# shichaoy/cube_slam

Hardware: AMD Instinct MI355X
Metric: frames/sec front-end (ORB extract + LSD+LBD lines + cuboid: Canny+DT+sweep+score+select) @640x480 (higher is better)
Workload: dtype f64

## Files before the change

cube_slam_amd/csrc/cuboid.hip:

```cpp
#include "common.h"

#include <algorithm>
#include <array>
#include <climits>
#include <cmath>
#include <vector>

namespace {

constexpr int ROLL_CAP = 8;
constexpr int RP_CAP = ROLL_CAP * ROLL_CAP;
constexpr int SWEEP_HB = 1024;
constexpr int NMS_TW = 64, NMS_TH = 16;
constexpr int DT_INIT = INT_MAX >> 2;
constexpr int DT_HV = 62587;
constexpr int DT_DIAG = 89738;
constexpr size_t DT_SERIAL_ROW_BYTES = 2 * 4 * sizeof(int);
constexpr double PI = 3.14159265358979323846;
constexpr int SC_LDS_BYTES = 160 * 1024;
constexpr int SC_LUT_N = 1024;
constexpr int SC_CTRL_BYTES = 64;
constexpr int SC_MAP_OFF = SC_CTRL_BYTES + 2048;
constexpr int SC_MAP_ENTRIES = (SC_LDS_BYTES - SC_MAP_OFF) / 2;
constexpr float SC_ESC_D = 244.0f;
// ... 737 lines not shown
                if (!BWD) tmp[((long)i * C + k) * 64 + lane] = t;
                else lbuf[(rows_done & 1) * WC + jcol[k]] = (float)t * scale;
            }
            if (BWD) { flush_store(); rows_done++; }
        }
    }
    if (BWD && rows_done > 0) {
        const float *lb = lbuf + ((rows_done - 1) & 1) * WC;
#pragma unroll
        for (int q = 0; q < C; q++) ob[q] = lb[q * 64 + lane];
        oi = 0;
        flush_store();
    }
}
template <int C>
__global__ void __launch_bounds__(256) cuboid_dt_wave(const Unit *units, int n_units, const uint8_t *emap, int *tmp_arena, const long *tmp_off, float *dist) {
    const int u = blockIdx.x * 4 + (threadIdx.x >> 6);
    if (u >= n_units) return;
    const Unit &U = units[u];
    int *tmp = tmp_arena + tmp_off[u];
    __shared__ float s_line[4][2 * 64 * C];
    dt_wave_pass<C, false>(U, emap + U.pix_off, tmp, nullptr, nullptr);
    __builtin_amdgcn_fence(__ATOMIC_SEQ_CST, "workgroup");
    dt_wave_pass<C, true>(U, nullptr, tmp, dist + U.pix_off, s_line[threadIdx.x >> 6]);
}

struct VPEntry { double vp[6]; double ang[6]; };

__global__ void __launch_bounds__(256) cuboid_vp(const Unit *units, const UnitDyn *ud, const FrameDyn *fd, const CamRP *cam, const double *yaw,
                                                 Opts o, const double *mangle, const double *mmid, VPEntry *vpt) {
    const Unit &U = units[blockIdx.y];
    const FrameDyn &D = fd[U.frame];
    const int n_rp = D.n_roll * D.n_pitch;
    const int e = blockIdx.x * 256 + threadIdx.x;
    if (e >= n_rp * D.n_yaw) return;
    const int rp = e / D.n_yaw, yi = e % D.n_yaw;
    const CamRP &C = cam[(long)U.frame * RP_CAP + rp];
    const double y = yaw[(long)U.frame * o.yaw_cap + yi];
    const double cy = cos(y), sy = sin(y);
    VPEntry E;
    {
        const double d[3][3] = {{cy, sy, 0}, {-sy, cy, 0}, {0, 0, 1}};
        for (int k = 0; k < 3; k++) {
            double r[3];
            for (int i = 0; i < 3; i++) {
                double s = C.KinvR[i * 3 + 0] * d[k][0];
                s = s + C.KinvR[i * 3 + 1] * d[k][1];
                s = s + C.KinvR[i * 3 + 2] * d[k][2];
                r[i] = s;
// ... 863 lines not shown
                U.roi_w = U.roi_r - U.roi_x; U.roi_h = U.roi_b - U.roi_y;
                if (U.roi_w <= 0 || U.roi_h <= 0 || U.roi_x + U.roi_w > width || U.roi_y + U.roi_h > height) { ctx->err = "box ROI outside the image"; return CS_ERR_BAD_ARG; }
                U.pix_off = P.pix_total; P.pix_total += ((long)U.roi_w * U.roi_h + 63) / 64 * 64;
                U.hyp_cap = rp_cap * o.yaw_cap * U.n_tops * 2;
                U.hyp_off = P.hyp_total; P.hyp_total += ((long)U.hyp_cap + 63) / 64 * 64;
                U.vp_off = (int)P.vp_total; P.vp_total += (long)rp_cap * o.yaw_cap;
                U.line_off = (int)P.line_rows; P.line_rows += std::min(fi[f].n_lines, CS_MAX_ROI_LINES);
                U.nms_off = P.n_nms; P.n_nms += ((U.roi_w + NMS_TW - 1) / NMS_TW) * ((U.roi_h + NMS_TH - 1) / NMS_TH);
                U.cc_off = P.n_cc; P.n_cc += (int)(((long)U.roi_w * U.roi_h + 4095) / 4096);
                U.hb_off = P.n_hb; P.n_hb += (U.hyp_cap + SWEEP_HB - 1) / SWEEP_HB;
                P.max_roi_w = std::max(P.max_roi_w, U.roi_w);
                P.max_cc_blocks = std::max(P.max_cc_blocks, (int)(((long)U.roi_w * U.roi_h + 4095) / 4096));
                P.units.push_back(U);
            }
        }
    P.max_vp_blocks = (rp_cap * o.yaw_cap + 255) / 256;
    P.n_units = (int)P.units.size();
    if (P.vp_total > INT_MAX || P.line_rows > INT_MAX) return CS_ERR_CAPACITY;
    return CS_OK;
}
static void plan_derived(Plan &P, int score_G) {
    const size_t n = P.units.size();
    P.wgmap.resize((size_t)P.n_nms + P.n_cc + P.n_hb);
    for (size_t u = 0; u < n; u++) {
        const Unit &U = P.units[u];
        const int e_nms = u + 1 < n ? P.units[u + 1].nms_off : P.n_nms, e_cc = u + 1 < n ? P.units[u + 1].cc_off : P.n_cc, e_hb = u + 1 < n ? P.units[u + 1].hb_off : P.n_hb;
        for (int k = U.nms_off; k < e_nms; k++) P.wgmap[(size_t)k] = (int)u;
        for (int k = U.cc_off; k < e_cc; k++) P.wgmap[(size_t)P.n_nms + k] = (int)u;
        for (int k = U.hb_off; k < e_hb; k++) P.wgmap[(size_t)P.n_nms + P.n_cc + k] = (int)u;
    }
    static const int CS_[] = {4, 5, 6, 8, 10, 12, 16, 20};
// ... 290 lines not shown
    for (const FrameInfo &fi_ : b->fi) ul_cap = std::max(ul_cap, std::min(fi_.n_lines, CS_MAX_ROI_LINES));
    const bool fork = !ctx->timing;
    hipStream_t side = ctx->stream;
    SideBranch branch{ctx};
    if (fork) {
        CS_HIP(ctx, ctx->aux_get(&side));
        if (!b->ev_fork) CS_HIP(ctx, hipEventCreateWithFlags(&b->ev_fork, hipEventDisableTiming));
        if (!b->ev_join) CS_HIP(ctx, hipEventCreateWithFlags(&b->ev_join, hipEventDisableTiming));
        CS_HIP(ctx, hipEventRecord(b->ev_fork, ctx->stream));
        branch.side = side;
        CS_HIP(ctx, hipStreamWaitEvent(side, b->ev_fork, 0));
    }
    CS_LAUNCH_ON(ctx, side, "cuboid_frame_prep", cuboid_frame_prep, dim3(b->n_frames), dim3(64), 0, b->d_fi, b->d_fd, b->d_cam, b->d_yaw, b->cal, b->o, b->d_lines_in, b->d_lines_al);
    CS_LAUNCH_ON(ctx, side, "cuboid_unit_lines", cuboid_unit_lines, dim3(U), dim3(64), sizeof(double) * 5 * (size_t)ul_cap, b->d_units, b->d_ud, b->d_fi, b->d_lines_al, b->d_mlines,
                 b->d_mangle, b->d_mmid, b->d_status, ul_cap);
    CS_LAUNCH_ON(ctx, side, "cuboid_vp", cuboid_vp, dim3(b->max_vp_blocks, U), dim3(256), 0, b->d_units, b->d_ud, b->d_fd, b->d_cam, b->d_yaw, b->o, b->d_mangle, b->d_mmid, b->d_vp);
    CS_HIP(ctx, hipGetLastError());
    if (fork) { CS_HIP(ctx, hipEventRecord(b->ev_join, side)); branch.joined = b->ev_join; }
    CS_HIP(ctx, hipMemsetAsync(b->d_emap, 0, (size_t)b->pix_total, ctx->stream));
    CS_LAUNCH(ctx, "cuboid_canny_nms", cuboid_canny_nms, dim3(b->n_nms), dim3(256), 0, b->d_units, b->d_wgmap, b->d_gray, b->W, b->H, b->d_emap,
              b->d_lab, b->o.canny_low, b->o.canny_high);
    CS_LAUNCH(ctx, "cuboid_canny_cc_local", cuboid_canny_cc_local, dim3(b->n_cc), dim3(256), 0, b->d_units, b->d_wgmap + b->n_nms, b->d_emap, b->d_lab);
    if (b->max_cc_blocks > 1)
        CS_LAUNCH(ctx, "cuboid_canny_cc_border", cuboid_canny_cc_border, dim3(U, 4), dim3(256), 0, b->d_units, b->d_emap, b->d_lab);
    CS_LAUNCH(ctx, "cuboid_canny_cc", cuboid_canny_cc, dim3(b->n_cc), dim3(256), 0, b->d_units, b->d_wgmap + b->n_nms, b->d_emap, b->d_lab);
    if (b->dt_C) {
        const dim3 g((U + 3) / 4), t(256);
        switch (b->dt_C) {
#define DTW_(c) case c: CS_LAUNCH(ctx, "cuboid_dt", cuboid_dt_wave<c>, g, t, 0, b->d_units, U, b->d_emap, b->d_dttmp, b->d_dttmp_off, b->d_dist); break;
            DTW_(4) DTW_(5) DTW_(6) DTW_(8) DTW_(10) DTW_(12) DTW_(16) DTW_(20)
#undef DTW_
        }
    } else if (b->max_roi_w <= 1024) {
        CS_LAUNCH(ctx, "cuboid_dt", cuboid_dt_block, dim3(U), dim3(64 * ((b->max_roi_w + 63) / 64)), 0, b->d_units, b->d_emap, b->d_dist);
    } else {
        const int wbuf = b->max_roi_w + 2;
        CS_LAUNCH(ctx, "cuboid_dt", cuboid_dt, dim3((U + 3) / 4), dim3(256), (size_t)wbuf * DT_SERIAL_ROW_BYTES, b->d_units, U, b->d_emap, b->d_dist, wbuf);
    }
    CS_HIP(ctx, branch.join());
    CS_HIP(ctx, hipMemsetAsync(b->d_vcount, 0, sizeof(int) * 2 * (size_t)U, ctx->stream));
    CS_LAUNCH(ctx, "cuboid_sweep_filter", cuboid_sweep_filter, dim3(b->n_hb), dim3(256), 0, b->d_units, b->d_wgmap + b->n_nms + b->n_cc, b->d_fd, b->o, b->d_vp,
              b->d_flag, b->d_vcount, b->d_vlist);
// ... 202 lines not shown
```

cube_slam_amd/csrc/lsd.hip:

```cpp
#include "common.h"
#include "glibc_sincosf.h"
#include "lsd_regions.h"

#include <cfloat>
#include <chrono>
#include <cmath>
#include <mutex>
#include <omp.h>
#include <vector>

namespace {
constexpr double NOTDEF = -1024.0, PI_ = 3.1415926535897932384626433832795, DEG_TO_RADS = PI_ / 180;
constexpr float NOTDEF_DEG = -1024.0f;
constexpr int KH = 3;

__host__ __device__ inline float fast_atan2f_(float y, float x) {
    const float p1 = 0.9997878412794807f * (float)(180 / PI_), p3 = -0.3258083974640975f * (float)(180 / PI_), p5 = 0.1555786518463281f * (float)(180 / PI_),
                p7 = -0.04432655554792128f * (float)(180 / PI_);
    float ax = fabsf(x), ay = fabsf(y), a, c, c2;
    if (ax >= ay) { c = ay / (ax + (float)DBL_EPSILON); c2 = c * c; a = (((p7 * c2 + p5) * c2 + p3) * c2 + p1) * c; }
    else { c = ax / (ay + (float)DBL_EPSILON); c2 = c * c; a = 90.f - (((p7 * c2 + p5) * c2 + p3) * c2 + p1) * c; }
    if (x < 0) a = 180.f - a;
    if (y < 0) a = 360.f - a;
    return a;
// ... 94 lines not shown
        }
    };
#pragma unroll
    for (int u = 0; u < AHEAD; u++) fetch(u, ca[u], cc[u]);
    for (int k0 = 0; k0 < total; k0 += G) {
#pragma unroll
        for (int u = 0; u < G; u++)
            if (k0 + u < total) { fetch(k0 + u + AHEAD, ca[(u + AHEAD) % G], cc[(u + AHEAD) % G]); row(k0 + u, u, ca[u], cc[u]); }
    }
    if (dy_last == h - 1 && y0 + LSD_ROWS >= h) {
        if (mine) { const long o = (frame_px + h - 1) * w + dx; modgrad[o] = 0; angles[o] = NOTDEF_DEG; }
        if (lane == 0) seg_cnt[(frame_px + h - 1) * seg_stride + strip] = 0;
    }
}
static_assert(EMIT_STRIPS == 4, "lsd_scan_blocks reads a segment's strip counts as one int4");
__global__ void __launch_bounds__(1024) lsd_scan_blocks(const int4 *in, int n, int *out, int *block_tot) {
    __shared__ int ws[16];
    const int i = blockIdx.x * 1024 + threadIdx.x, lane = threadIdx.x & 63, wave = threadIdx.x >> 6;
    int v = 0;
    if (i < n) { const int4 q = in[i]; v = q.x + q.y + q.z + q.w; }
    const int sc = wave_incl_scan(v, lane);
    if (lane == 63) ws[wave] = sc;
    __syncthreads();
    int base = 0;
    for (int k = 0; k < wave; k++) base += ws[k];
    if (i < n) out[i] = base + sc - v;
    if (threadIdx.x == 1023) block_tot[blockIdx.x] = base + sc;
}
__global__ void __launch_bounds__(1024) lsd_scan_add(int *out, int n, const int *block_tot) {
    __shared__ int ws[16];
    int part = 0;
    for (int k = threadIdx.x; k < (int)blockIdx.x; k += 1024) part += block_tot[k];
    for (int d = 32; d > 0; d >>= 1) part += __shfl_xor(part, d);
    if ((threadIdx.x & 63) == 0) ws[threadIdx.x >> 6] = part;
    __syncthreads();
    int base = 0;
    for (int k = 0; k < 16; k++) base += ws[k];
    const int i = blockIdx.x * 1024 + threadIdx.x;
    if (i < n) out[i] += base;
    if (blockIdx.x == gridDim.x - 1 && threadIdx.x == 0) out[n] = base + block_tot[blockIdx.x];
}
template <bool PIX> __global__ void __launch_bounds__(EMIT_COLS) lsd_emit(const double *modgrad, const float *angles, int w, int h, const int *seg_base, int *c_addr, float *c_deg, float2 *c_cs, double *c_mod, float *fre ) {
    constexpr int NW = EMIT_COLS / 64, LW = EMIT_COLS + 2;
    __shared__ float s_ang[(EMIT_ROWS + 2) * LW];
    __shared__ int s_list[EMIT_ROWS * EMIT_COLS], s_need[PIX ? EMIT_ROWS * EMIT_COLS : 1];
    __shared__ int wc[EMIT_ROWS][NW], s_base[EMIT_ROWS], n_need;
    const int tid = threadIdx.x, x0 = blockIdx.x * EMIT_COLS, y0 = blockIdx.y * EMIT_ROWS;
    const long frame_row = (long)blockIdx.z * h;
    for (int i = tid; i < (EMIT_ROWS + 2) * LW; i += EMIT_COLS) {
        const int yy = y0 - 1 + i / LW, xx = x0 - 1 + i % LW;
        s_ang[i] = xx >= 0 && xx < w && yy >= 0 && yy < h ? angles[(frame_row + yy) * w + xx] : NOTDEF_DEG;
    }
    if (tid < EMIT_ROWS && y0 + tid < h) s_base[tid] = seg_base[(frame_row + y0 + tid) * gridDim.x + blockIdx.x];
    if (tid == 0) n_need = 0;
// ... 424 lines not shown
}

static int lsd_run(cs_ctx *ctx, cs_lsd *l, int with_lbd) {
    if (!ctx || !l || l->n_frames < 1) return CS_ERR_BAD_ARG;
    CS_HIP(ctx, hipSetDevice(ctx->device));
    const int W = l->W, H = l->H, w = l->w, h = l->h, F = l->n_frames;
    l->have_desc = false;
    const char *mode = getenv("CUBESLAM_LSD_REGIONS");
    if (!mode || !*mode) mode = l->region_stage == CS_LSD_REGIONS_HOST ? "host" : l->region_stage == CS_LSD_REGIONS_WAVE_PER_FRAME ? "seq" : l->region_stage == CS_LSD_REGIONS_BACKLOG ? "wlk" : (F >= 512 ? "seq" : "host");
    const int grp_p = strcmp(mode, "wlk") == 0 ? 65 : 0;
    const bool device_mode = strcmp(mode, "seq") == 0 || grp_p;
    l->scaled_kept = !device_mode;
    const int nbx = l->nbx, nsx = l->nsx, n_seg = F * h * nbx;
    CS_LAUNCH(ctx, "lsd_gradient", lsd_maps, dim3(nsx * ((h + LSD_ROWS - 1) / LSD_ROWS), 1, F), dim3(64), 0, l->d_gray, W, H, w, h, l->gk, (MapTabs{l->d_xofs, l->d_yofs, l->d_ax, l->d_ay}), l->threshold,
              l->d_mod, l->d_ang, l->d_seg_cnt, nbx * EMIT_STRIPS, device_mode ? (double *)nullptr : l->d_scaled);
    const int nblk = (n_seg + 1023) / 1024;
    CS_LAUNCH(ctx, "lsd_scan", lsd_scan_blocks, dim3(nblk), dim3(1024), 0, reinterpret_cast<const int4 *>(l->d_seg_cnt), n_seg, l->d_seg_base, l->d_blk_tot);
    CS_LAUNCH(ctx, "lsd_scan", lsd_scan_add, dim3(nblk), dim3(1024), 0, l->d_seg_base, n_seg, l->d_blk_tot);
    l->frame_base.assign((size_t)F + 1, 0);
    CS_HIP(ctx, hipMemcpy2DAsync(l->frame_base.data(), sizeof(int), l->d_seg_base, sizeof(int) * (size_t)h * nbx, sizeof(int), (size_t)F + 1, hipMemcpyDeviceToHost, ctx->stream));
    CS_HIP(ctx, hipStreamSynchronize(ctx->stream));
    const size_t total = (size_t)l->frame_base[F];
    int r;
    if (total > l->ccap) {
        void *old[] = {l->d_caddr, l->d_cdeg, l->d_ccs, l->d_cmod};
        for (void *q : old) cs_dfree(ctx, q);
        l->d_caddr = nullptr; l->d_cdeg = nullptr; l->d_ccs = nullptr; l->d_cmod = nullptr; l->ccap = 0;
        const size_t cap = total + total / 16 + 4096;
        r = cs_dalloc(ctx, &l->d_caddr, cap); if (r) return r;
        r = cs_dalloc(ctx, &l->d_cdeg, cap); if (r) return r;
        r = cs_dalloc(ctx, &l->d_ccs, cap); if (r) return r;
        l->ccap = cap;
    }
// ... 160 lines not shown
    std::vector<float> ax((size_t)l->w * 2), ay((size_t)l->h * 2);
    auto fl = [](double v) { int i = (int)v; return i - (i > v); };
    for (int dx = 0; dx < l->w; dx++) { float fx = (float)((dx + 0.5) * sx - 0.5); int s = fl(fx); fx -= s; if (s < 0) { fx = 0; s = 0; } if (s >= width - 1) { fx = 0; s = width - 1; } xofs[dx] = s; ax[dx * 2] = 1.f - fx; ax[dx * 2 + 1] = fx; }
    for (int dy = 0; dy < l->h; dy++) { float fy = (float)((dy + 0.5) * sx - 0.5); int s = fl(fy); fy -= s; if (s < 0) { fy = 0; s = 0; } if (s >= height - 1) { fy = 0; s = height - 1; } yofs[dy] = s; ay[dy * 2] = 1.f - fy; ay[dy * 2 + 1] = fy; }
    const size_t N = (size_t)width * height * max_frames, n = (size_t)l->w * l->h * max_frames;
#define A_(call) do { int r__ = (call); if (r__ != CS_OK) { cs_lsd_destroy(ctx, l); return r__; } } while (0)
    l->pix_bytes = (n * 4 + 64 + 255) / 256 * 256;
    A_(cs_dalloc(ctx, &l->d_gray, N)); A_(cs_dalloc(ctx, &l->d_tmp, N + n)); l->d_scaled = l->d_tmp + N;
    A_(cs_dalloc(ctx, &l->d_mod, n)); A_(cs_dalloc(ctx, &l->d_ang, n));
    A_(cs_dalloc(ctx, &l->d_xofs, xofs.size())); A_(cs_dalloc(ctx, &l->d_yofs, yofs.size())); A_(cs_dalloc(ctx, &l->d_ax, ax.size())); A_(cs_dalloc(ctx, &l->d_ay, ay.size()));
    l->nsx = (l->w + LSD_COLS - 1) / LSD_COLS; l->nbx = (l->nsx + EMIT_STRIPS - 1) / EMIT_STRIPS;
    for (int d0 = 0; d0 < l->w; d0 += LSD_COLS)
        if (std::min(xofs[std::min(d0 + LSD_COLS, l->w - 1)] + 1, width - 1) - xofs[d0] >= LSD_SPAN) { cs_lsd_destroy(ctx, l); return CS_ERR_BAD_ARG; }
    const size_t n_seg = (size_t)max_frames * l->h * l->nbx;
    A_(cs_dalloc(ctx, &l->d_seg_cnt, n_seg * EMIT_STRIPS)); A_(cs_dalloc(ctx, &l->d_seg_base, n_seg + 1));
    A_(cs_dalloc(ctx, &l->d_blk_tot, (n_seg + 1023) / 1024 + 1));
    { hipError_t e = hipMemsetAsync(l->d_seg_cnt, 0, n_seg * EMIT_STRIPS * sizeof(int), ctx->stream); if (e != hipSuccess) { cs_lsd_destroy(ctx, l); return CS_ERR_HIP; } }
    A_(cs_h2d(ctx, l->d_xofs, xofs.data(), xofs.size())); A_(cs_h2d(ctx, l->d_yofs, yofs.data(), yofs.size()));
    A_(cs_h2d(ctx, l->d_ax, ax.data(), ax.size())); A_(cs_h2d(ctx, l->d_ay, ay.data(), ay.size()));
#undef A_
    { hipError_t e = hipStreamSynchronize(ctx->stream); if (e != hipSuccess) { cs_lsd_destroy(ctx, l); return CS_ERR_HIP; } }
    *out = l;
    return CS_OK;
}

int cs_lsd_detect(cs_ctx *ctx, cs_lsd *l, const uint8_t *gray, int n_frames, int stride, cs_keyline *out, int cap, int *counts) {
    if (!out || !counts || cap < 1) return CS_ERR_BAD_ARG;
    int r = lsd_upload(ctx, l, gray, n_frames, stride); if (r) return r;
    r = lsd_run(ctx, l, 0); if (r) return r;
    int status = CS_OK;
    for (int f = 0; f < n_frames; f++) {
// ... 128 lines not shown
```

cube_slam_amd/csrc/lsd_regions.hip:

```cpp
#include "common.h"

#include <cfloat>
#include <climits>
#include <cmath>
#include <vector>

#include "lsd_regions.h"
#include "lsd_rg_seq.h"
#include "lsd_rg_wlk.h"

namespace {
constexpr int PAD_PX = 272, PAD_LIST = 272, PAD_RECT = 34;
constexpr double PI_ = rg::PI_, LOG_EPS = 0.0, LSD_SCALE = 0.8;
struct AngMap { int w, h; const float *deg; };

__device__ __forceinline__ double rg_log_gamma_windschitl(double x) { return 0.918938533204673 + (x - 0.5) * log(x) - x + 0.5 * x * log(x * sinh(1 / x) + 1 / (810.0 * pow(x, 6.0))); }
__device__ double rg_log_gamma(double x) {
    if (x > 15.0) return rg_log_gamma_windschitl(x);
    const double q[7] = {75122.6331530, 80916.6278952, 36308.2951477, 8687.24529705, 1168.92649479, 83.8676043424, 2.50662827511};
    double a = (x + 0.5) * log(x + 5.5) - (x + 5.5), b = 0;
    for (int n = 0; n < 7; ++n) { a -= log(x + double(n)); b += q[n] * pow(x, double(n)); }
    return a + log(b);
}
#ifndef RG_IMPROVE_WAVES
#ifndef RG_IMPROVE_WAVES
#define RG_IMPROVE_WAVES 3
#endif
#endif
constexpr int LG_N = 32768;
__global__ void __launch_bounds__(256) lsd_rg_lgamma_table(double *t) { const int i = blockIdx.x * 256 + threadIdx.x; if (i < LG_N) t[i] = i > 0 ? rg_log_gamma(double(i)) : 0.0; }
__device__ __forceinline__ double rg_lgam_int(int x, const double *lgt) { return x < LG_N ? lgt[x] : rg_log_gamma_windschitl(double(x)); }
__device__ double rg_nfa(int n, int k, double p, double LOG_NT, const double *lgt) {
    if (n == 0 || k == 0) return -LOG_NT;
    if (n == k) return -LOG_NT - double(n) * log10(p);
    const double p_term = p / (1 - p);
    const double log1term = (double(n) + 1) - rg_lgam_int(k + 1, lgt) - rg_lgam_int(n - k + 1, lgt) + double(k) * log(p) + double(n - k) * log(1.0 - p);
    double term = exp(log1term);
    const double RELATIVE_ERROR_FACTOR = 100.0;
    auto double_equal = [&](double a, double b) { if (a == b) return true; double abs_diff = fabs(a - b), aa = fabs(a), bb = fabs(b); double abs_max = aa > bb ? aa : bb; if (abs_max < DBL_MIN) abs_max = DBL_MIN; return (abs_diff / abs_max) <= (RELATIVE_ERROR_FACTOR * DBL_EPSILON); };
    if (double_equal(term, 0)) { if (k > n * p) return -log1term / 2.30258509299404568402 - LOG_NT; else return -LOG_NT; }
    double bin_tail = term;
    const double tolerance = 0.1;
    for (int i = k + 1; i <= n; ++i) {
        const double bin_term = double(n - i + 1) / double(i), mult_term = bin_term * p_term;
        term *= mult_term;
        bin_tail += term;
        if (bin_term < 1) {
// ... 239 lines not shown
        return;
    }
    for (;;) {
        int t = 0;
        if (lane == 0) t = rgw::lds_add(&mail.head, 1);
        t = __builtin_amdgcn_readfirstlane(t);
        bool quit = false;
        while (__builtin_amdgcn_readfirstlane(rgw::lds_ld(&mail.ring_tick[t % NS])) != t + 1) {
            if (__builtin_amdgcn_readfirstlane(rgw::lds_ld(&mail.walkers_done)) == WK && __builtin_amdgcn_readfirstlane(rgw::lds_ld(&mail.tail)) <= t) { quit = true; break; }
            __builtin_amdgcn_s_sleep(4);
        }
        if (quit) break;
        rgw::serve_ticket<rgs::Wave, NS>(B, mail, t);
    }
}
__global__ void __launch_bounds__(1024) lsd_rg_cand_scan(const int *cand_cnt, int F, int *cand_base) {
    __shared__ int part[1024];
    const int t = threadIdx.x, per = (F + 1023) / 1024;
    int sum = 0;
    for (int k = 0; k < per; k++) { const int f = t * per + k; if (f < F) sum += cand_cnt[f]; }
    part[t] = sum;
    __syncthreads();
    for (int d = 1; d < 1024; d <<= 1) { const int v = t >= d ? part[t - d] : 0; __syncthreads(); part[t] += v; __syncthreads(); }
    int run = part[t] - sum;
    for (int k = 0; k < per; k++) { const int f = t * per + k; if (f < F) { cand_base[f] = run; run += cand_cnt[f]; } }
    if (t == 1023) cand_base[F] = part[1023];
}
constexpr uint8_t HAS_DEFERRED = 2;
template <class E, bool REDO> __device__ __forceinline__ void lsd_rg_improve_body(const SeqParams &P, const int *cand_base, int n_cand, const E &nfa, float4 *line, uint8_t *has, unsigned long long *counters) {
    const int base = (blockIdx.x * 4 + (threadIdx.x >> 6)) * 8, lane = threadIdx.x & 63, grp = lane >> 3, sub = lane & 7;
    if (base >= n_cand) return;
    const int mine = base + grp;
    bool on = mine < n_cand;
    if (REDO) {
        on = on && has[mine] == HAS_DEFERRED;
        if (!__any(on)) return;
    }
    auto frame_of = [&](int wv) { int lo = 0, hi = P.F; while (hi - lo > 1) { const int mid = (lo + hi) >> 1; if (cand_base[mid] <= wv) lo = mid; else hi = mid; } return lo; };
    auto load_rect = [&](int wv, int f, rg::Rect &rec) {
        const double *o = P.rect + (size_t)f * P.rect_stride + (size_t)(wv - cand_base[f]) * 12;
        rec.x1 = o[0]; rec.y1 = o[1]; rec.x2 = o[2]; rec.y2 = o[3]; rec.width = o[4]; rec.x = o[5]; rec.y = o[6]; rec.theta = o[7]; rec.dx = o[8]; rec.dy = o[9]; rec.prec = o[10]; rec.p = o[11];
    };
    auto emit = [&](int wv, rg::Rect rec, double log_nfa) {
        const bool ok = log_nfa > LOG_EPS;
        if (ok) {
            rec.x1 += 0.5; rec.y1 += 0.5; rec.x2 += 0.5; rec.y2 += 0.5;
            rec.x1 /= LSD_SCALE; rec.y1 /= LSD_SCALE; rec.x2 /= LSD_SCALE; rec.y2 /= LSD_SCALE;
            line[wv] = make_float4(float(rec.x1), float(rec.y1), float(rec.x2), float(rec.y2));
        }
        has[wv] = ok ? 1 : 0;
    };
    const int f1 = frame_of(on ? mine : n_cand - 1);
// ... 4 lines not shown
    {
        RectSpan S; S.set(r1, P.h);
        const float *deg = P.ang + (size_t)f1 * P.w * P.h;
        int tot = 0, alg[1] = {0};
        if (on)
            for (int y = S.y_first + sub; y <= S.y_hi; y += 8) {
                int lx, rx;
                if (!S.row(y, P.w, lx, rx)) continue;
                tot += rx - lx + 1;
                rg_row_count<1>(deg + (size_t)y * P.w, lx, rx, 0, 1, r1.theta, &r1.prec, alg);
            }
        for (int off = 1; off < 8; off <<= 1) { tot += __shfl_xor(tot, off); alg[0] += __shfl_xor(alg[0], off); }
        log1 = nfa(tot, alg[0], r1.p, miss1);
    }
    if (on && sub == 0) { if (miss1) has[mine] = HAS_DEFERRED; else if (log1 > LOG_EPS) emit(mine, r1, log1); }
    int n_deferred = __popcll(__ballot(on && sub == 0 && miss1));
    unsigned long long todo = __ballot(on && sub == 0 && !miss1 && !(log1 > LOG_EPS));
    while (todo) {
        const int l = __ffsll((long long)todo) - 1;
        todo &= todo - 1;
        const int wv = base + (l >> 3), f = __shfl(f1, l);
        const double first = __shfl(log1, l);
        rg::Rect rec;
        load_rect(wv, f, rec);
        const AngMap Fr = {P.w, P.h, P.ang + (size_t)f * P.w * P.h};
        bool missed = false;
        const double log_nfa = rg_rect_improve(Fr, rec, nfa, lane, first, missed);
        if (missed) { n_deferred++; if (lane == 0) has[wv] = HAS_DEFERRED; }
        else if (lane == 0) emit(wv, rec, log_nfa);
    }
    if (!REDO && lane == 0) atomicAdd(counters, (unsigned long long)(min(8, n_cand - base) - n_deferred) | (unsigned long long)n_deferred << 32);
}
__global__ void __launch_bounds__(256) __attribute__((amdgpu_waves_per_eu(4, 4))) lsd_rg_improve(SeqParams P, const int *cand_base, int n_cand, const double *nfa_table, int nfa_nmax, float4 *line, uint8_t *has, unsigned long long *counters) {
    lsd_rg_improve_body<NfaTable, false>(P, cand_base, n_cand, NfaTable{nfa_table, nfa_nmax}, line, has, counters);
}
__global__ void __launch_bounds__(256) __attribute__((amdgpu_waves_per_eu(RG_IMPROVE_WAVES, RG_IMPROVE_WAVES))) lsd_rg_improve_deferred(SeqParams P, const int *cand_base, int n_cand, const double *lgt, float4 *line, uint8_t *has) {
    lsd_rg_improve_body<NfaDirect, true>(P, cand_base, n_cand, NfaDirect{rg_log_nt(P.w, P.h), lgt}, line, has, nullptr);
}
__global__ void __launch_bounds__(256) lsd_rg_nfa_probe(const int *t, int m, const double *nfa_table, int nfa_nmax, int w, int h, const double *lgt, double *out) {
    const int i = blockIdx.x * 256 + threadIdx.x;
    if (i >= m) return;
    const int n = t[3 * i], k = t[3 * i + 1], j = t[3 * i + 2];
    const double p = ldexp(1.0, -(3 + j));
    bool miss = false;
    const double v = NfaTable{nfa_table, nfa_nmax}(n, k, p, miss);
    out[2 * i] = miss ? __longlong_as_double(0x7ff8000000000000LL) : v;
    out[2 * i + 1] = rg_nfa(n, k, p, rg_log_nt(w, h), lgt);
}
}

struct LsdSeq {
    int F = 0, w = 0, h = 0; int cand_cap = 0; size_t cap_lines = 0;
    float *d_pix = nullptr; bool pix_borrowed = false;
    rgl::Ent *d_elist = nullptr; float *d_ang32 = nullptr; int *d_order = nullptr;
    int *d_glist = nullptr, *d_cand_cnt = nullptr, *d_cand_base = nullptr, *d_status = nullptr, *d_frame_base = nullptr;
    double *d_rect = nullptr, *d_lgt = nullptr, *d_nfa = nullptr;
    unsigned long long *d_counters = nullptr; cs_pinned<unsigned long long> h_counters; long nfa_counts[2] = {0, 0};
    uint8_t *d_has = nullptr;
    float4 *d_line = nullptr;
    cs_pinned<int> h_base, h_status; cs_pinned<uint8_t> h_has; cs_pinned<float4> h_line;
};
static int lsd_nfa_bound() {
    const char *e = getenv("CUBESLAM_LSD_NFA_NMAX");
    return e ? std::max(0, std::min(NFA_NMAX, atoi(e))) : NFA_NMAX;
}
void lsd_seq_destroy(cs_ctx *ctx, LsdSeq *r) {
    if (!r) return;
    void *ptrs[] = {r->d_elist, r->d_ang32, r->d_order, r->pix_borrowed ? nullptr : r->d_pix, r->d_glist, r->d_cand_cnt, r->d_cand_base, r->d_status, r->d_frame_base, r->d_rect, r->d_lgt, r->d_nfa, r->d_counters, r->d_has, r->d_line};
    for (void *p : ptrs) cs_dfree(ctx, p);
    r->h_base.release(); r->h_status.release(); r->h_has.release(); r->h_line.release(); r->h_counters.release();
    delete r;
}
int lsd_seq_run(cs_ctx *ctx, LsdSeq **handle, int F, int w, int h, const float *d_ang, const double *d_mod, const int *d_caddr, const float *d_cdeg, const float2 *d_ccs, const int *frame_base,
                std::vector<std::vector<float>> &lines, long *stats ,
                void (*before_seq)(void *), void (*after_seq)(void *), void *gate_arg ,
                int grp_p ,
                int waves_per_workgroup ,
                void *scratch, size_t scratch_bytes ,
                bool pix_ready ,
                bool walk_bg ) {
    LsdSeq *r = *handle;
    if (w > 0xffff || h > 0x7fff) return CS_ERR_CAPACITY;
    int max_ne = 0;
// ... 71 lines not shown
                B.list = r->d_elist + (size_t)c0 * list_stride; B.list_cap = std::min(S.list_cap, rgl::CAP); B.rect = r->d_rect + (size_t)c0 * rect_stride; B.cand_cap = r->cand_cap; B.cand_cnt = r->d_cand_cnt + c0; B.status = r->d_status + 4 * (size_t)c0;
                B.min_reg_size = S.min_reg_size; B.max_iters = (int)std::min<size_t>(64 * npx, 0x7fffffff);
            }
            int wk = 1, nw = 8, acc = 1;
            if (const char *e = getenv("CUBESLAM_LSD_WLK")) sscanf(e, "%d,%d,%d", &wk, &nw, &acc);
            const int bps = (L.waves_per_slice + wk - 1) / wk, groups = L.n_slices * bps;
#define WLK_(WK, NW, AC) else if (wk == WK && nw == NW && acc == AC) CS_LAUNCH(ctx, "lsd_rg_wlk", (lsd_rg_wlk<WK, NW, AC>), dim3(groups), dim3(64 * NW), 0, L, bps)
            if (false) {}
            WLK_(1, 8, 1); WLK_(1, 8, 2); WLK_(2, 8, 1); WLK_(8, 16, 1);
            else { ctx->err = "CUBESLAM_LSD_WLK: no such shape (walkers,waves,accepts)"; return CS_ERR_BAD_ARG; }
#undef WLK_
        }
    } else if (walk_bg) {
        CS_HIP(ctx, ctx->bg_begin());
        CS_LAUNCH_BG(ctx, "lsd_rg_seq", lsd_rg_seq, dim3((F + wpb - 1) / wpb), dim3(64 * wpb), 0, S);
        CS_LAUNCH_BG(ctx, "lsd_rg_cand_scan", lsd_rg_cand_scan, dim3(1), dim3(1024), 0, r->d_cand_cnt, F, r->d_cand_base);
        CS_HIP(ctx, hipMemcpyAsync(r->h_base.p, r->d_cand_base, ((size_t)F + 1) * sizeof(int), hipMemcpyDeviceToHost, ctx->bg_stream));
        CS_HIP(ctx, hipMemcpyAsync(r->h_status.p, r->d_status, (size_t)F * 4 * sizeof(int), hipMemcpyDeviceToHost, ctx->bg_stream));
        CS_HIP(ctx, ctx->bg_end());
    } else
    CS_LAUNCH(ctx, "lsd_rg_seq", lsd_rg_seq, dim3((F + wpb - 1) / wpb), dim3(64 * wpb), 0, S);
    if (grp || !walk_bg) {
        CS_LAUNCH(ctx, "lsd_rg_cand_scan", lsd_rg_cand_scan, dim3(1), dim3(1024), 0, r->d_cand_cnt, F, r->d_cand_base);
        RA_(cs_d2h(ctx, r->h_base.p, r->d_cand_base, (size_t)F + 1));
        RA_(cs_d2h(ctx, r->h_status.p, r->d_status, (size_t)F * 4));
        CS_HIP(ctx, hipStreamSynchronize(ctx->stream));
    }
    if (after_seq) after_seq(gate_arg);
    long grows = 0, fetches = 0, nreg = 0;
    bool bad = false;
    for (int f = 0; f < F; f++) { grows += r->h_status.p[4 * f]; bad = bad || r->h_status.p[4 * f + 1] != 0; nreg += r->h_status.p[4 * f + 2]; fetches += r->h_status.p[4 * f + 3]; }
    const int n_cand = r->h_base.p[F];
    if (stats) { stats[0] = grows; stats[1] = fetches; stats[2] = n_cand; stats[3] = nreg; }
    if (bad) return CS_ERR_CAPACITY;
    lines.assign((size_t)F, {});
    r->nfa_counts[0] = r->nfa_counts[1] = 0;
    if (n_cand == 0) return CS_OK;
    if ((size_t)n_cand > r->cap_lines) {
        cs_dfree(ctx, r->d_line); cs_dfree(ctx, r->d_has);
        r->d_line = nullptr; r->d_has = nullptr; r->cap_lines = 0;
        const size_t cap = (size_t)n_cand + n_cand / 4 + 1024;
        RA_(cs_dalloc(ctx, &r->d_line, cap)); RA_(cs_dalloc(ctx, &r->d_has, cap));
        r->cap_lines = cap;
    }
    RA_(r->h_has.reserve(ctx, (size_t)n_cand)); RA_(r->h_line.reserve(ctx, (size_t)n_cand));
    CS_HIP(ctx, hipMemsetAsync(r->d_counters, 0, sizeof(unsigned long long), ctx->stream));
    CS_LAUNCH(ctx, "lsd_rg_improve", lsd_rg_improve, dim3((n_cand + 31) / 32), dim3(256), 0, S, r->d_cand_base, n_cand, r->d_nfa, nfa_nmax ? nfa_nmax : -1, r->d_line, r->d_has, r->d_counters);
    CS_LAUNCH(ctx, "lsd_rg_improve_deferred", lsd_rg_improve_deferred, dim3((n_cand + 31) / 32), dim3(256), 0, S, r->d_cand_base, n_cand, r->d_lgt, r->d_line, r->d_has);
    RA_(cs_d2h(ctx, r->h_has.p, r->d_has, (size_t)n_cand));
    RA_(cs_d2h(ctx, r->h_line.p, r->d_line, (size_t)n_cand));
    RA_(cs_d2h(ctx, r->h_counters.p, r->d_counters, (size_t)1));
    CS_HIP(ctx, hipStreamSynchronize(ctx->stream));
    r->nfa_counts[0] = (long)(r->h_counters.p[0] & 0xffffffffull); r->nfa_counts[1] = (long)(r->h_counters.p[0] >> 32);
#undef RA_
#pragma omp parallel for schedule(static) num_threads(std::max(1, std::min(ctx->host_threads, F)))
    for (int f = 0; f < F; f++)
        for (int k = r->h_base.p[f]; k < r->h_base.p[f + 1]; k++)
            if (r->h_has.p[k]) { const float4 v = r->h_line.p[k]; lines[f].push_back(v.x); lines[f].push_back(v.y); lines[f].push_back(v.z); lines[f].push_back(v.w); }
    return CS_OK;
}
int lsd_seq_nfa_probe(cs_ctx *ctx, LsdSeq *r, int m, const int *triples, double *out, long *counters) {
    if (!r || !r->d_nfa || m < 0 || (m > 0 && (!triples || !out))) return CS_ERR_BAD_ARG;
    for (int i = 0; i < m; i++) if (triples[3 * i] < 0 || triples[3 * i + 1] < 0 || triples[3 * i + 1] > triples[3 * i] || triples[3 * i + 2] < 0 || triples[3 * i + 2] >= NFA_NP) return CS_ERR_BAD_ARG;
// ... 12 lines not shown
```

Before: 30210.

## Shrink workgroups to single waves and compact deferred LSD candidates

Several kernels (cuboid DT, VP, LSD scans, candidate scan, region improve) are relaunched as single-wave or smaller workgroups, so block-level barriers and shared-memory scans become wave scans. The deferred-refinement pass now reads a compacted list of deferred candidate indices, built with an atomic counter, and runs a grid-stride loop over it instead of scanning every candidate. Other changes: rg_nfa is force-inlined and the deferred kernel's waves-per-EU setting goes up. The aim is less idle-lane and barrier overhead and less wasted work in the deferred pass, at the cost of more, smaller workgroups and an extra index buffer.

```diff
diff --git a/cube_slam_amd/csrc/cuboid.hip b/cube_slam_amd/csrc/cuboid.hip
--- a/cube_slam_amd/csrc/cuboid.hip
+++ b/cube_slam_amd/csrc/cuboid.hip
@@ -775,25 +775,25 @@
     }
 }
 template <int C>
-__global__ void __launch_bounds__(256) cuboid_dt_wave(const Unit *units, int n_units, const uint8_t *emap, int *tmp_arena, const long *tmp_off, float *dist) {
-    const int u = blockIdx.x * 4 + (threadIdx.x >> 6);
+__global__ void __launch_bounds__(64) cuboid_dt_wave(const Unit *units, int n_units, const uint8_t *emap, int *tmp_arena, const long *tmp_off, float *dist) {
+    const int u = blockIdx.x;
     if (u >= n_units) return;
     const Unit &U = units[u];
     int *tmp = tmp_arena + tmp_off[u];
-    __shared__ float s_line[4][2 * 64 * C];
+    __shared__ float s_line[2 * 64 * C];
     dt_wave_pass<C, false>(U, emap + U.pix_off, tmp, nullptr, nullptr);
     __builtin_amdgcn_fence(__ATOMIC_SEQ_CST, "workgroup");
-    dt_wave_pass<C, true>(U, nullptr, tmp, dist + U.pix_off, s_line[threadIdx.x >> 6]);
+    dt_wave_pass<C, true>(U, nullptr, tmp, dist + U.pix_off, s_line);
 }
 
 struct VPEntry { double vp[6]; double ang[6]; };
 
-__global__ void __launch_bounds__(256) cuboid_vp(const Unit *units, const UnitDyn *ud, const FrameDyn *fd, const CamRP *cam, const double *yaw,
+__global__ void __launch_bounds__(64) cuboid_vp(const Unit *units, const UnitDyn *ud, const FrameDyn *fd, const CamRP *cam, const double *yaw,
                                                  Opts o, const double *mangle, const double *mmid, VPEntry *vpt) {
     const Unit &U = units[blockIdx.y];
     const FrameDyn &D = fd[U.frame];
     const int n_rp = D.n_roll * D.n_pitch;
-    const int e = blockIdx.x * 256 + threadIdx.x;
+    const int e = blockIdx.x * 64 + threadIdx.x;
     if (e >= n_rp * D.n_yaw) return;
     const int rp = e / D.n_yaw, yi = e % D.n_yaw;
     const CamRP &C = cam[(long)U.frame * RP_CAP + rp];
@@ -1687,7 +1687,7 @@
                 P.units.push_back(U);
             }
         }
-    P.max_vp_blocks = (rp_cap * o.yaw_cap + 255) / 256;
+    P.max_vp_blocks = (rp_cap * o.yaw_cap + 63) / 64;
     P.n_units = (int)P.units.size();
     if (P.vp_total > INT_MAX || P.line_rows > INT_MAX) return CS_ERR_CAPACITY;
     return CS_OK;
@@ -2008,7 +2008,7 @@
     CS_LAUNCH_ON(ctx, side, "cuboid_frame_prep", cuboid_frame_prep, dim3(b->n_frames), dim3(64), 0, b->d_fi, b->d_fd, b->d_cam, b->d_yaw, b->cal, b->o, b->d_lines_in, b->d_lines_al);
     CS_LAUNCH_ON(ctx, side, "cuboid_unit_lines", cuboid_unit_lines, dim3(U), dim3(64), sizeof(double) * 5 * (size_t)ul_cap, b->d_units, b->d_ud, b->d_fi, b->d_lines_al, b->d_mlines,
                  b->d_mangle, b->d_mmid, b->d_status, ul_cap);
-    CS_LAUNCH_ON(ctx, side, "cuboid_vp", cuboid_vp, dim3(b->max_vp_blocks, U), dim3(256), 0, b->d_units, b->d_ud, b->d_fd, b->d_cam, b->d_yaw, b->o, b->d_mangle, b->d_mmid, b->d_vp);
+    CS_LAUNCH_ON(ctx, side, "cuboid_vp", cuboid_vp, dim3(b->max_vp_blocks, U), dim3(64), 0, b->d_units, b->d_ud, b->d_fd, b->d_cam, b->d_yaw, b->o, b->d_mangle, b->d_mmid, b->d_vp);
     CS_HIP(ctx, hipGetLastError());
     if (fork) { CS_HIP(ctx, hipEventRecord(b->ev_join, side)); branch.joined = b->ev_join; }
     CS_HIP(ctx, hipMemsetAsync(b->d_emap, 0, (size_t)b->pix_total, ctx->stream));
@@ -2019,7 +2019,7 @@
         CS_LAUNCH(ctx, "cuboid_canny_cc_border", cuboid_canny_cc_border, dim3(U, 4), dim3(256), 0, b->d_units, b->d_emap, b->d_lab);
     CS_LAUNCH(ctx, "cuboid_canny_cc", cuboid_canny_cc, dim3(b->n_cc), dim3(256), 0, b->d_units, b->d_wgmap + b->n_nms, b->d_emap, b->d_lab);
     if (b->dt_C) {
-        const dim3 g((U + 3) / 4), t(256);
+        const dim3 g(U), t(64);
         switch (b->dt_C) {
 #define DTW_(c) case c: CS_LAUNCH(ctx, "cuboid_dt", cuboid_dt_wave<c>, g, t, 0, b->d_units, U, b->d_emap, b->d_dttmp, b->d_dttmp_off, b->d_dist); break;
             DTW_(4) DTW_(5) DTW_(6) DTW_(8) DTW_(10) DTW_(12) DTW_(16) DTW_(20)
diff --git a/cube_slam_amd/csrc/lsd.hip b/cube_slam_amd/csrc/lsd.hip
--- a/cube_slam_amd/csrc/lsd.hip
+++ b/cube_slam_amd/csrc/lsd.hip
@@ -132,30 +132,32 @@
     }
 }
 static_assert(EMIT_STRIPS == 4, "lsd_scan_blocks reads a segment's strip counts as one int4");
-__global__ void __launch_bounds__(1024) lsd_scan_blocks(const int4 *in, int n, int *out, int *block_tot) {
-    __shared__ int ws[16];
-    const int i = blockIdx.x * 1024 + threadIdx.x, lane = threadIdx.x & 63, wave = threadIdx.x >> 6;
-    int v = 0;
-    if (i < n) { const int4 q = in[i]; v = q.x + q.y + q.z + q.w; }
-    const int sc = wave_incl_scan(v, lane);
-    if (lane == 63) ws[wave] = sc;
-    __syncthreads();
-    int base = 0;
-    for (int k = 0; k < wave; k++) base += ws[k];
-    if (i < n) out[i] = base + sc - v;
-    if (threadIdx.x == 1023) block_tot[blockIdx.x] = base + sc;
-}
-__global__ void __launch_bounds__(1024) lsd_scan_add(int *out, int n, const int *block_tot) {
-    __shared__ int ws[16];
+constexpr int SCAN_BLOCK = 1024, SCAN_THREADS = 256, SCAN_TURNS = SCAN_BLOCK / SCAN_THREADS;
+__global__ void __launch_bounds__(SCAN_THREADS) lsd_scan_blocks(const int4 *in, int n, int *out, int *block_tot) {
+    __shared__ int ws[SCAN_THREADS / 64];
+    const int lane = threadIdx.x & 63, i0 = blockIdx.x * SCAN_BLOCK + (threadIdx.x >> 6) * (64 * SCAN_TURNS) + lane;
+    int v[SCAN_TURNS], run = 0;
+#pragma unroll
+    for (int k = 0; k < SCAN_TURNS; k++) { const int i = i0 + k * 64; v[k] = 0; if (i < n) { const int4 q = in[i]; v[k] = q.x + q.y + q.z + q.w; } }
+#pragma unroll
+    for (int k = 0; k < SCAN_TURNS; k++) { const int sc = wave_incl_scan(v[k], lane); v[k] = run + sc - v[k]; run += __shfl(sc, 63); }
+    int total;
+    const int base = block_waves_before<SCAN_THREADS / 64>(run, ws, &total);
+#pragma unroll
+    for (int k = 0; k < SCAN_TURNS; k++) { const int i = i0 + k * 64; if (i < n) out[i] = base + v[k]; }
+    if (threadIdx.x == 0) block_tot[blockIdx.x] = total;
+}
+__global__ void __launch_bounds__(SCAN_THREADS) lsd_scan_add(int *out, int n, const int *block_tot) {
+    __shared__ int ws[SCAN_THREADS / 64];
     int part = 0;
-    for (int k = threadIdx.x; k < (int)blockIdx.x; k += 1024) part += block_tot[k];
+    for (int k = threadIdx.x; k < (int)blockIdx.x; k += SCAN_THREADS) part += block_tot[k];
     for (int d = 32; d > 0; d >>= 1) part += __shfl_xor(part, d);
     if ((threadIdx.x & 63) == 0) ws[threadIdx.x >> 6] = part;
     __syncthreads();
     int base = 0;
-    for (int k = 0; k < 16; k++) base += ws[k];
-    const int i = blockIdx.x * 1024 + threadIdx.x;
-    if (i < n) out[i] += base;
+    for (int k = 0; k < SCAN_THREADS / 64; k++) base += ws[k];
+#pragma unroll
+    for (int k = 0; k < SCAN_TURNS; k++) { const int i = blockIdx.x * SCAN_BLOCK + k * SCAN_THREADS + threadIdx.x; if (i < n) out[i] += base; }
     if (blockIdx.x == gridDim.x - 1 && threadIdx.x == 0) out[n] = base + block_tot[blockIdx.x];
 }
 template <bool PIX> __global__ void __launch_bounds__(EMIT_COLS) lsd_emit(const double *modgrad, const float *angles, int w, int h, const int *seg_base, int *c_addr, float *c_deg, float2 *c_cs, double *c_mod, float *fre ) {
@@ -610,9 +612,9 @@
     const int nbx = l->nbx, nsx = l->nsx, n_seg = F * h * nbx;
     CS_LAUNCH(ctx, "lsd_gradient", lsd_maps, dim3(nsx * ((h + LSD_ROWS - 1) / LSD_ROWS), 1, F), dim3(64), 0, l->d_gray, W, H, w, h, l->gk, (MapTabs{l->d_xofs, l->d_yofs, l->d_ax, l->d_ay}), l->threshold,
               l->d_mod, l->d_ang, l->d_seg_cnt, nbx * EMIT_STRIPS, device_mode ? (double *)nullptr : l->d_scaled);
-    const int nblk = (n_seg + 1023) / 1024;
-    CS_LAUNCH(ctx, "lsd_scan", lsd_scan_blocks, dim3(nblk), dim3(1024), 0, reinterpret_cast<const int4 *>(l->d_seg_cnt), n_seg, l->d_seg_base, l->d_blk_tot);
-    CS_LAUNCH(ctx, "lsd_scan", lsd_scan_add, dim3(nblk), dim3(1024), 0, l->d_seg_base, n_seg, l->d_blk_tot);
+    const int nblk = (n_seg + SCAN_BLOCK - 1) / SCAN_BLOCK;
+    CS_LAUNCH(ctx, "lsd_scan", lsd_scan_blocks, dim3(nblk), dim3(SCAN_THREADS), 0, reinterpret_cast<const int4 *>(l->d_seg_cnt), n_seg, l->d_seg_base, l->d_blk_tot);
+    CS_LAUNCH(ctx, "lsd_scan", lsd_scan_add, dim3(nblk), dim3(SCAN_THREADS), 0, l->d_seg_base, n_seg, l->d_blk_tot);
     l->frame_base.assign((size_t)F + 1, 0);
     CS_HIP(ctx, hipMemcpy2DAsync(l->frame_base.data(), sizeof(int), l->d_seg_base, sizeof(int) * (size_t)h * nbx, sizeof(int), (size_t)F + 1, hipMemcpyDeviceToHost, ctx->stream));
     CS_HIP(ctx, hipStreamSynchronize(ctx->stream));
@@ -803,7 +805,7 @@
         if (std::min(xofs[std::min(d0 + LSD_COLS, l->w - 1)] + 1, width - 1) - xofs[d0] >= LSD_SPAN) { cs_lsd_destroy(ctx, l); return CS_ERR_BAD_ARG; }
     const size_t n_seg = (size_t)max_frames * l->h * l->nbx;
     A_(cs_dalloc(ctx, &l->d_seg_cnt, n_seg * EMIT_STRIPS)); A_(cs_dalloc(ctx, &l->d_seg_base, n_seg + 1));
-    A_(cs_dalloc(ctx, &l->d_blk_tot, (n_seg + 1023) / 1024 + 1));
+    A_(cs_dalloc(ctx, &l->d_blk_tot, (n_seg + SCAN_BLOCK - 1) / SCAN_BLOCK + 1));
     { hipError_t e = hipMemsetAsync(l->d_seg_cnt, 0, n_seg * EMIT_STRIPS * sizeof(int), ctx->stream); if (e != hipSuccess) { cs_lsd_destroy(ctx, l); return CS_ERR_HIP; } }
     A_(cs_h2d(ctx, l->d_xofs, xofs.data(), xofs.size())); A_(cs_h2d(ctx, l->d_yofs, yofs.data(), yofs.size()));
     A_(cs_h2d(ctx, l->d_ax, ax.data(), ax.size())); A_(cs_h2d(ctx, l->d_ay, ay.data(), ay.size()));
diff --git a/cube_slam_amd/csrc/lsd_regions.hip b/cube_slam_amd/csrc/lsd_regions.hip
--- a/cube_slam_amd/csrc/lsd_regions.hip
+++ b/cube_slam_amd/csrc/lsd_regions.hip
@@ -23,14 +23,12 @@
     return a + log(b);
 }
 #ifndef RG_IMPROVE_WAVES
-#ifndef RG_IMPROVE_WAVES
-#define RG_IMPROVE_WAVES 3
-#endif
+#define RG_IMPROVE_WAVES 4
 #endif
 constexpr int LG_N = 32768;
 __global__ void __launch_bounds__(256) lsd_rg_lgamma_table(double *t) { const int i = blockIdx.x * 256 + threadIdx.x; if (i < LG_N) t[i] = i > 0 ? rg_log_gamma(double(i)) : 0.0; }
 __device__ __forceinline__ double rg_lgam_int(int x, const double *lgt) { return x < LG_N ? lgt[x] : rg_log_gamma_windschitl(double(x)); }
-__device__ double rg_nfa(int n, int k, double p, double LOG_NT, const double *lgt) {
+__device__ __forceinline__ double rg_nfa(int n, int k, double p, double LOG_NT, const double *lgt) {
     if (n == 0 || k == 0) return -LOG_NT;
     if (n == k) return -LOG_NT - double(n) * log10(p);
     const double p_term = p / (1 - p);
@@ -300,28 +298,19 @@
         rgw::serve_ticket<rgs::Wave, NS>(B, mail, t);
     }
 }
-__global__ void __launch_bounds__(1024) lsd_rg_cand_scan(const int *cand_cnt, int F, int *cand_base) {
-    __shared__ int part[1024];
-    const int t = threadIdx.x, per = (F + 1023) / 1024;
+__global__ void __launch_bounds__(64) lsd_rg_cand_scan(const int *cand_cnt, int F, int *cand_base) {
+    const int lane = threadIdx.x, per = (F + 63) / 64, f0 = lane * per, f1 = min(F, f0 + per);
     int sum = 0;
-    for (int k = 0; k < per; k++) { const int f = t * per + k; if (f < F) sum += cand_cnt[f]; }
-    part[t] = sum;
-    __syncthreads();
-    for (int d = 1; d < 1024; d <<= 1) { const int v = t >= d ? part[t - d] : 0; __syncthreads(); part[t] += v; __syncthreads(); }
-    int run = part[t] - sum;
-    for (int k = 0; k < per; k++) { const int f = t * per + k; if (f < F) { cand_base[f] = run; run += cand_cnt[f]; } }
-    if (t == 1023) cand_base[F] = part[1023];
+    for (int f = f0; f < f1; f++) sum += cand_cnt[f];
+    const int inc = wave_incl_scan(sum, lane);
+    int run = inc - sum;
+    for (int f = f0; f < f1; f++) { cand_base[f] = run; run += cand_cnt[f]; }
+    if (lane == 63) cand_base[F] = inc;
 }
 constexpr uint8_t HAS_DEFERRED = 2;
-template <class E, bool REDO> __device__ __forceinline__ void lsd_rg_improve_body(const SeqParams &P, const int *cand_base, int n_cand, const E &nfa, float4 *line, uint8_t *has, unsigned long long *counters) {
-    const int base = (blockIdx.x * 4 + (threadIdx.x >> 6)) * 8, lane = threadIdx.x & 63, grp = lane >> 3, sub = lane & 7;
-    if (base >= n_cand) return;
-    const int mine = base + grp;
-    bool on = mine < n_cand;
-    if (REDO) {
-        on = on && has[mine] == HAS_DEFERRED;
-        if (!__any(on)) return;
-    }
+constexpr int RG_DEFERRED_GRID = 1024;
+template <class E> __device__ __forceinline__ unsigned long long lsd_rg_improve_wave(const SeqParams &P, const int *cand_base, int n_cand, const E &nfa, float4 *line, uint8_t *has, int mine, bool on) {
+    const int lane = threadIdx.x & 63, sub = lane & 7;
     auto frame_of = [&](int wv) { int lo = 0, hi = P.F; while (hi - lo > 1) { const int mid = (lo + hi) >> 1; if (cand_base[mid] <= wv) lo = mid; else hi = mid; } return lo; };
     auto load_rect = [&](int wv, int f, rg::Rect &rec) {
         const double *o = P.rect + (size_t)f * P.rect_stride + (size_t)(wv - cand_base[f]) * 12;
@@ -356,28 +345,42 @@
         log1 = nfa(tot, alg[0], r1.p, miss1);
     }
     if (on && sub == 0) { if (miss1) has[mine] = HAS_DEFERRED; else if (log1 > LOG_EPS) emit(mine, r1, log1); }
-    int n_deferred = __popcll(__ballot(on && sub == 0 && miss1));
+    unsigned long long deferred = __ballot(on && sub == 0 && miss1);
     unsigned long long todo = __ballot(on && sub == 0 && !miss1 && !(log1 > LOG_EPS));
     while (todo) {
         const int l = __ffsll((long long)todo) - 1;
         todo &= todo - 1;
-        const int wv = base + (l >> 3), f = __shfl(f1, l);
+        const int wv = __shfl(mine, l), f = __shfl(f1, l);
         const double first = __shfl(log1, l);
         rg::Rect rec;
         load_rect(wv, f, rec);
         const AngMap Fr = {P.w, P.h, P.ang + (size_t)f * P.w * P.h};
         bool missed = false;
         const double log_nfa = rg_rect_improve(Fr, rec, nfa, lane, first, missed);
-        if (missed) { n_deferred++; if (lane == 0) has[wv] = HAS_DEFERRED; }
+        if (missed) { deferred |= 1ull << l; if (lane == 0) has[wv] = HAS_DEFERRED; }
         else if (lane == 0) emit(wv, rec, log_nfa);
     }
-    if (!REDO && lane == 0) atomicAdd(counters, (unsigned long long)(min(8, n_cand - base) - n_deferred) | (unsigned long long)n_deferred << 32);
-}
-__global__ void __launch_bounds__(256) __attribute__((amdgpu_waves_per_eu(4, 4))) lsd_rg_improve(SeqParams P, const int *cand_base, int n_cand, const double *nfa_table, int nfa_nmax, float4 *line, uint8_t *has, unsigned long long *counters) {
-    lsd_rg_improve_body<NfaTable, false>(P, cand_base, n_cand, NfaTable{nfa_table, nfa_nmax}, line, has, counters);
-}
-__global__ void __launch_bounds__(256) __attribute__((amdgpu_waves_per_eu(RG_IMPROVE_WAVES, RG_IMPROVE_WAVES))) lsd_rg_improve_deferred(SeqParams P, const int *cand_base, int n_cand, const double *lgt, float4 *line, uint8_t *has) {
-    lsd_rg_improve_body<NfaDirect, true>(P, cand_base, n_cand, NfaDirect{rg_log_nt(P.w, P.h), lgt}, line, has, nullptr);
+    return deferred;
+}
+__global__ void __launch_bounds__(64) __attribute__((amdgpu_waves_per_eu(4, 4))) lsd_rg_improve(SeqParams P, const int *cand_base, int n_cand, const double *nfa_table, int nfa_nmax, float4 *line, uint8_t *has, unsigned long long *counters, int *deferred) {
+    const int base = blockIdx.x * 8, lane = threadIdx.x;
+    if (base >= n_cand) return;
+    const int mine = base + (lane >> 3);
+    const unsigned long long dm = lsd_rg_improve_wave(P, cand_base, n_cand, NfaTable{nfa_table, nfa_nmax}, line, has, mine, mine < n_cand);
+    const int nd = __popcll(dm);
+    unsigned long long old = 0;
+    if (lane == 0) old = atomicAdd(counters, (unsigned long long)(min(8, n_cand - base) - nd) | (unsigned long long)nd << 32);
+    if (nd == 0) return;
+    const int slot = __shfl(int(old >> 32), 0);
+    if (dm >> lane & 1) deferred[slot + wave_rank(dm, lane)] = mine;
+}
+__global__ void __launch_bounds__(64) __attribute__((amdgpu_waves_per_eu(RG_IMPROVE_WAVES, RG_IMPROVE_WAVES))) lsd_rg_improve_deferred(SeqParams P, const int *cand_base, int n_cand, const double *lgt, float4 *line, uint8_t *has, const unsigned long long *counters, const int *deferred) {
+    const int n = int(*counters >> 32), grp = threadIdx.x >> 3;
+    const NfaDirect nfa{rg_log_nt(P.w, P.h), lgt};
+    for (int t = blockIdx.x; t * 8 < n; t += gridDim.x) {
+        const int k = t * 8 + grp;
+        lsd_rg_improve_wave(P, cand_base, n_cand, nfa, line, has, k < n ? deferred[k] : 0, k < n);
+    }
 }
 __global__ void __launch_bounds__(256) lsd_rg_nfa_probe(const int *t, int m, const double *nfa_table, int nfa_nmax, int w, int h, const double *lgt, double *out) {
     const int i = blockIdx.x * 256 + threadIdx.x;
@@ -399,6 +402,7 @@
     double *d_rect = nullptr, *d_lgt = nullptr, *d_nfa = nullptr;
     unsigned long long *d_counters = nullptr; cs_pinned<unsigned long long> h_counters; long nfa_counts[2] = {0, 0};
     uint8_t *d_has = nullptr;
+    int *d_deferred = nullptr;
     float4 *d_line = nullptr;
     cs_pinned<int> h_base, h_status; cs_pinned<uint8_t> h_has; cs_pinned<float4> h_line;
 };
@@ -408,7 +412,7 @@
 }
 void lsd_seq_destroy(cs_ctx *ctx, LsdSeq *r) {
     if (!r) return;
-    void *ptrs[] = {r->d_elist, r->d_ang32, r->d_order, r->pix_borrowed ? nullptr : r->d_pix, r->d_glist, r->d_cand_cnt, r->d_cand_base, r->d_status, r->d_frame_base, r->d_rect, r->d_lgt, r->d_nfa, r->d_counters, r->d_has, r->d_line};
+    void *ptrs[] = {r->d_elist, r->d_ang32, r->d_order, r->pix_borrowed ? nullptr : r->d_pix, r->d_glist, r->d_cand_cnt, r->d_cand_base, r->d_status, r->d_frame_base, r->d_rect, r->d_lgt, r->d_nfa, r->d_counters, r->d_has, r->d_deferred, r->d_line};
     for (void *p : ptrs) cs_dfree(ctx, p);
     r->h_base.release(); r->h_status.release(); r->h_has.release(); r->h_line.release(); r->h_counters.release();
     delete r;
@@ -510,14 +514,14 @@
     } else if (walk_bg) {
         CS_HIP(ctx, ctx->bg_begin());
         CS_LAUNCH_BG(ctx, "lsd_rg_seq", lsd_rg_seq, dim3((F + wpb - 1) / wpb), dim3(64 * wpb), 0, S);
-        CS_LAUNCH_BG(ctx, "lsd_rg_cand_scan", lsd_rg_cand_scan, dim3(1), dim3(1024), 0, r->d_cand_cnt, F, r->d_cand_base);
+        CS_LAUNCH_BG(ctx, "lsd_rg_cand_scan", lsd_rg_cand_scan, dim3(1), dim3(64), 0, r->d_cand_cnt, F, r->d_cand_base);
         CS_HIP(ctx, hipMemcpyAsync(r->h_base.p, r->d_cand_base, ((size_t)F + 1) * sizeof(int), hipMemcpyDeviceToHost, ctx->bg_stream));
         CS_HIP(ctx, hipMemcpyAsync(r->h_status.p, r->d_status, (size_t)F * 4 * sizeof(int), hipMemcpyDeviceToHost, ctx->bg_stream));
         CS_HIP(ctx, ctx->bg_end());
     } else
     CS_LAUNCH(ctx, "lsd_rg_seq", lsd_rg_seq, dim3((F + wpb - 1) / wpb), dim3(64 * wpb), 0, S);
     if (grp || !walk_bg) {
-        CS_LAUNCH(ctx, "lsd_rg_cand_scan", lsd_rg_cand_scan, dim3(1), dim3(1024), 0, r->d_cand_cnt, F, r->d_cand_base);
+        CS_LAUNCH(ctx, "lsd_rg_cand_scan", lsd_rg_cand_scan, dim3(1), dim3(64), 0, r->d_cand_cnt, F, r->d_cand_base);
         RA_(cs_d2h(ctx, r->h_base.p, r->d_cand_base, (size_t)F + 1));
         RA_(cs_d2h(ctx, r->h_status.p, r->d_status, (size_t)F * 4));
         CS_HIP(ctx, hipStreamSynchronize(ctx->stream));
@@ -533,16 +537,17 @@
     r->nfa_counts[0] = r->nfa_counts[1] = 0;
     if (n_cand == 0) return CS_OK;
     if ((size_t)n_cand > r->cap_lines) {
-        cs_dfree(ctx, r->d_line); cs_dfree(ctx, r->d_has);
-        r->d_line = nullptr; r->d_has = nullptr; r->cap_lines = 0;
+        cs_dfree(ctx, r->d_line); cs_dfree(ctx, r->d_has); cs_dfree(ctx, r->d_deferred);
+        r->d_line = nullptr; r->d_has = nullptr; r->d_deferred = nullptr; r->cap_lines = 0;
         const size_t cap = (size_t)n_cand + n_cand / 4 + 1024;
-        RA_(cs_dalloc(ctx, &r->d_line, cap)); RA_(cs_dalloc(ctx, &r->d_has, cap));
+        RA_(cs_dalloc(ctx, &r->d_line, cap)); RA_(cs_dalloc(ctx, &r->d_has, cap)); RA_(cs_dalloc(ctx, &r->d_deferred, cap));
         r->cap_lines = cap;
     }
     RA_(r->h_has.reserve(ctx, (size_t)n_cand)); RA_(r->h_line.reserve(ctx, (size_t)n_cand));
     CS_HIP(ctx, hipMemsetAsync(r->d_counters, 0, sizeof(unsigned long long), ctx->stream));
-    CS_LAUNCH(ctx, "lsd_rg_improve", lsd_rg_improve, dim3((n_cand + 31) / 32), dim3(256), 0, S, r->d_cand_base, n_cand, r->d_nfa, nfa_nmax ? nfa_nmax : -1, r->d_line, r->d_has, r->d_counters);
-    CS_LAUNCH(ctx, "lsd_rg_improve_deferred", lsd_rg_improve_deferred, dim3((n_cand + 31) / 32), dim3(256), 0, S, r->d_cand_base, n_cand, r->d_lgt, r->d_line, r->d_has);
+    const int n_waves = (n_cand + 7) / 8;
+    CS_LAUNCH(ctx, "lsd_rg_improve", lsd_rg_improve, dim3(n_waves), dim3(64), 0, S, r->d_cand_base, n_cand, r->d_nfa, nfa_nmax ? nfa_nmax : -1, r->d_line, r->d_has, r->d_counters, r->d_deferred);
+    CS_LAUNCH(ctx, "lsd_rg_improve_deferred", lsd_rg_improve_deferred, dim3(std::min(n_waves, RG_DEFERRED_GRID)), dim3(64), 0, S, r->d_cand_base, n_cand, r->d_lgt, r->d_line, r->d_has, r->d_counters, r->d_deferred);
     RA_(cs_d2h(ctx, r->h_has.p, r->d_has, (size_t)n_cand));
     RA_(cs_d2h(ctx, r->h_line.p, r->d_line, (size_t)n_cand));
     RA_(cs_d2h(ctx, r->h_counters.p, r->d_counters, (size_t)1));
```

Result: no change. 30160 (-0.2%).
